# ZihanLiao/pytorch-kaldi-resnet

Measured on AMD Instinct MI355X. Metric: utterances/sec (300-frame x 80 fbank, bs256/GPU), ResNet-34 + AAM-softmax training step, higher is better.
Workload: dtype f32 (operands as 2 fp16 terms of value x 2^k, 3 cross products, f32 accumulate); 1 GPU; BASELINE configs[1]: ResNet-34 + AAM-softmax (m 0.2, s 30), 1211 speakers, 300-frame x 80 fbank, per-GPU batch 256, fwd+CE+bwd+SGD(0.9, wd 5e-4); global_batch=256, frames=300, feat_dim=80, parallelism=dp1, launch=hipGraph replay (1 graph), mfma=f16x3

## Files before the change

### include/spkhip.h

```cpp
#ifndef SPKHIP_H
#define SPKHIP_H
#include <stddef.h>
#ifdef __cplusplus
extern "C" {
#endif

int spk_version(void);
const char* spk_last_error(void);
int spk_build_flags(void);

#define SPK_IN_AFFINE_RELU 1
#define SPK_EPI_AFFINE 2
#define SPK_EPI_ADD 4
#define SPK_EPI_RELU 8
#define SPK_EPI_STATS 16
#define SPK_IN_BNBWD 64
#define SPK_EPI_BNBWD 32

#define SPK_CONV_WS 128
#define SPK_CONV_PIPE 1024

#define SPK_CONV_M16 (1 << 17)

#define SPK_WGRAD_GROUPS 2048
// ... 34 lines not shown

int spk_conv_wgrad_limits(int WN, int* max_halo_pix , int* max_tile_pix );
size_t spk_conv_wgrad_workspace(int nsplit, int ksize, int Cin, int Cout);
int spk_conv3x3_c32_stream(const float* in, const float* wpk, float* out, const float* in_scale, const float* in_shift, float* stats,
                           int B, int H, int W, int flags, const unsigned* in_amax, unsigned* out_amax, int nblocks, void* stream);
int spk_conv1x1_stream(const float* in, const float* wpk, float* out, const float* in_scale, const float* in_shift,
                       const float* epi_add, const unsigned* add_mask, const float* bn_raw, const unsigned* bn_mask,
                       const float* bn4, float* stats, long long P, int C, int flags, const unsigned* in_amax, unsigned* out_amax,
                       int nblocks, void* stream);
int spk_conv1x1_stream_rows(int nblocks, int C);
int spk_wgrad_reduce(const float* partial, float* dw, int nslab, int ksize, int Cin, int Cout, int accumulate, void* stream);
int spk_conv_wgrad(const float* x, const float* dy, float* dw, float* partial, const float* in_scale,
                   const float* in_shift, int B, int IH, int IW, int Cin, int OH, int OW, int Cout, int ksize, int stride,
                   int TH, int TW, int WN, int nsplit, int flags, int accumulate, int split , const unsigned* dy_amax , const unsigned* x_amax , void* stream);

#define SPK_PTR_ADD_MASK 1
#define SPK_PTR_BN_MASK 2
#define SPK_PTR_IN_MASK 4
#define SPK_PTR_IN_ACT 8
#define SPK_PTR_BN_ACT 16
#define SPK_PTR_SIDE_DZ 32
int spk_conv_variant_of(int MT, int NT, int split, int flags, int ptrs);
int spk_wgrad_variant_of(int ksize, int stride, int TH, int TW, int WN, int split, int flags);

int spk_stem_fwd_blocks(int B, int F, int T);
int spk_stem_conv_fwd(const float* x, const float* w, float* out, float* stats, const float* epi_scale,
                      const float* epi_shift, int B, int F, int T, int flags,
                      unsigned* amax_out , void* stream);
int spk_stem_conv_fwd_len(const float* x, const float* w, float* out, float* stats, const float* epi_scale,
                          const float* epi_shift, int B, int F, int T, int flags, unsigned* amax_out, const int* len ,
                          void* stream);
int spk_stem_wgrad_blocks(int B, int F, int T);
int spk_stem_conv_wgrad(const float* x, const float* draw, float* dw, float* partial, int B, int F, int T,
                        int accumulate, void* stream);
int spk_stem_stats(const float* x, const float* w, float* stats, int B, int F, int T, void* stream);
int spk_stem_fwd_apply(const float* x, const float* w, const float* scale, const float* shift, float* raw_out, float* act_out,
                       unsigned* mask_out, unsigned* amax_out, int B, int F, int T, void* stream);
int spk_stem_bwd_wgrad(const float* x, const float* d, const float* raw, const float* mean, const float* invstd,
                       const float* scale, const float* shift, const float* coef, float* dw, float* partial, int B, int F, int T,
                       int accumulate, void* stream);

int spk_bn_stats_blocks(long long N, int C);
int spk_bn_stats_partial(const float* x, float* partial , long long N, int C, void* stream);
size_t spk_bn_finalize_workspace(int nblk, int C);
int spk_bn_finalize(const float* partial, int nblk, int C, double count, const float* gamma, const float* beta,
                    float* running_mean, float* running_var, long long* num_batches_tracked, float* mean, float* invstd,
// ... 221 lines not shown
```

### pytorch-kaldi-resnet_amd/csrc/conv_kernel.h

```cpp
#pragma once
#include "spk_common.h"
#include <type_traits>

#ifndef STAGE_U
#define STAGE_U 4
#endif
#ifndef CONV_NT
#define CONV_NT 3
#endif
static __device__ __forceinline__ void conv_st(float* p, f32x4 v) {
    if constexpr ((CONV_NT & 1) != 0) __builtin_nontemporal_store(v, (f32x4*)p);
    else *(f32x4*)p = v;
}
template <int BIT>
static __device__ __forceinline__ f32x4 conv_ld(const float* p) {
    if constexpr ((CONV_NT & BIT) != 0) return __builtin_nontemporal_load((const f32x4*)p);
    else return *(const f32x4*)p;
}
#ifndef STAGE_U2
#define STAGE_U2 2
#endif
#ifndef STAGE_U2_C32
#define STAGE_U2_C32 4
#endif

#define SPK_SPLIT_CK 16
template <int SPLIT, int CKP = SPK_SPLIT_CK>
struct ConvCfg {
    static_assert(CKP == SPK_SPLIT_CK || (SPLIT == 3 && CKP == 32), "plane width: 16, or 32 in the f16x3 mode");
    static constexpr int NTERM = SPLIT == 3 ? 2 : 3;
    static constexpr int MAXSUM = SPLIT == 9 ? 4 : (SPLIT == 6 ? 2 : 1);
    static constexpr int CK = SPLIT ? CKP : 32;
    static constexpr int TPP = CK / 4;
    static constexpr int PPP = 256 / TPP;
    static constexpr int KG = CK / 16;
    static constexpr int LP4 = SPLIT ? (NTERM * CK * 2 + 16) / 16 : 9;
};

struct ConvArgs {
    const float* in;
    const float* wpk;
    float* out;
    const float* in_scale;
    const float* in_shift;
    const float* epi_scale;
    const float* epi_shift;
// ... 38 lines not shown
           (a.in_act ? SPK_PTR_IN_ACT : 0) | (a.bn_act ? SPK_PTR_BN_ACT : 0) | (a.side_dz ? SPK_PTR_SIDE_DZ : 0);
}

#define PIPE_D 3
#ifndef PIPE16_D
#define PIPE16_D 3
#endif
#ifndef PIPE16_D_CONV
#define PIPE16_D_CONV 3
#endif
#ifndef PIPE_VPM
#define PIPE_VPM 6
#endif
#ifdef CONV_STAMPS
#define CONV_STAMP_BLOCKS 4096
static __device__ unsigned long long g_conv_stamps[CONV_STAMP_BLOCKS][16];
#define STAMP(i) do { if (threadIdx.x == 0 && blockIdx.x < CONV_STAMP_BLOCKS) g_conv_stamps[blockIdx.x][i] = __builtin_amdgcn_s_memtime(); } while (0)
#else
#define STAMP(i) do { } while (0)
#endif
#define SPK_FL_ADDMASK (1 << 20)
#define SPK_FL_BNMASK (1 << 21)
#define SPK_FL_INMASK (1 << 22)
template <int MT, int NT, bool BNBWD, int SPLIT, bool PIPE, bool BITS = false, bool PRE = false, bool M16 = false, int FL = -1, int CKP = SPK_SPLIT_CK>
static __device__ __forceinline__ void conv_body(const ConvArgs& a) {
    using Cfg = ConvCfg<SPLIT, CKP>;
    static_assert(CKP == SPK_SPLIT_CK || (BNBWD && !PIPE), "32-channel planes: the fused BatchNorm-backward form of conv_mfma_kernel");
    constexpr int CK = Cfg::CK, TPP = Cfg::TPP, PPP = Cfg::PPP, LP4 = Cfg::LP4, NTERM = Cfg::NTERM;
    static_assert(!M16 || (PIPE && !BNBWD && SPLIT == 3), "M16: the pipelined f16x3 kernel with a plain or pair input");
    extern __shared__ __attribute__((aligned(16))) float lds[];
    const int tid = threadIdx.x, lane = tid & 63;
    const int wave = __builtin_amdgcn_readfirstlane(tid >> 6);
    const int r = lane & 31, h = lane >> 5;
    auto pix_of_row16 = [](int row) {
        const int q = (row + 12) & 15;
        return ((q & 7) << 1) | (q >> 3);
    };
    float sig = 1.f, inv_sig = 1.f, inv_wsig = 1.f;
    if constexpr (SPLIT == 3) {
        sig = a.in_amax ? spk_sigma_from_amax_bits(*a.in_amax) : a.in_sigma;
        inv_sig = 1.f / sig;
        inv_wsig = 1.f / spk_sigma_from_amax_bits(*a.w_amax);
    }
    float side_mx = 0.f;

    int bid = blockIdx.x;
    {
        const int n = a.nblocks, q = n >> 3, rr = n & 7, xcd = bid & 7, slot = bid >> 3;
        bid = (xcd < rr ? xcd * (q + 1) : rr * (q + 1) + (xcd - rr) * q) + slot;
    }
// ... 77 lines not shown
            dst[0] = t0;
            dst[CK / 4] = t1;
        }
    };
    auto store_px_q = [&](float* plane, int p, int qd, f32x4 w) {
        if constexpr (SPLIT == 0) {
            *(f32x4*)(plane + p * (LP4 * 4) + qd * 4) = w;
        } else if constexpr (SPLIT == 3) {
            uint2 t0, t1;
            split2h(w, sig, t0, t1);
            store_pair_q(plane, p, qd, t0, t1);
        } else {
            uint2 t0, t1, t2;
            split3(w, t0, t1, t2);
            uint2* dst = (uint2*)plane + p * (LP4 * 2) + qd;
            dst[0] = t0;
            dst[CK / 4] = t1;
            dst[CK / 2] = t2;
        }
    };
    auto store_pair = [&](float* plane, int p, uint2 t0, uint2 t1) { store_pair_q(plane, p, quad, t0, t1); };
    auto store_px = [&](float* plane, int p, f32x4 w) { store_px_q(plane, p, quad, w); };

    auto stage_chunk_wide = [&](int ch) {
        const int tppk = TPP * a.kc;
        const int qk = tid & (tppk - 1);
        const int pl = qk / TPP, qd = qk & (TPP - 1);
        const int prowk = tid / tppk, pppk = 256 / tppk;
        const int c = (ch * a.kc + pl) * CK + qd * 4;
        float* ldsp = lds + pl * plane_floats;
        f32x4 sc = {1.f, 1.f, 1.f, 1.f}, sh = {0.f, 0.f, 0.f, 0.f};
        if (flags & SPK_IN_AFFINE_RELU) {
            sc = *(const f32x4*)(a.in_scale + c);
            sh = *(const f32x4*)(a.in_shift + c);
        }
        constexpr int U = STAGE_U;
        for (int base = prowk; base < halo_pix; base += pppk * U) {
            f32x4 v[U];
            bool inb[U];
#pragma unroll
            for (int u = 0; u < U; ++u) {
                int p = base + pppk * u;
                p = p < halo_pix ? p : halo_pix - 1;
                const int hy = (int)__umulhi((unsigned)p, a.halo_w_magic);
                const int hx = p - hy * a.halo_w;
                const int iy = iy0 + hy, ix = ix0 + hx;
                inb[u] = iy >= 0 && iy < a.IH && ix >= 0 && ix < a.IW;
                const unsigned pi = inb[u] ? (unsigned)((iy * a.IWp + ix) * a.ips) : pi_safe_p;
                v[u] = *(const f32x4*)(img_in_p + pi * (unsigned)a.Cin + (unsigned)c);
            }
#pragma unroll
            for (int u = 0; u < U; ++u) {
                const int p = base + pppk * u;
                f32x4 w = v[u];
                if (flags & SPK_IN_AFFINE_RELU) {
                    w = w * sc + sh;
                    w[0] = fmaxf(w[0], 0.f);
                    w[1] = fmaxf(w[1], 0.f);
                    w[2] = fmaxf(w[2], 0.f);
                    w[3] = fmaxf(w[3], 0.f);
                }
                if (!inb[u]) w = (f32x4){0.f, 0.f, 0.f, 0.f};
                if constexpr (SPLIT == 3) {
                    if (flags & SPK_IN_PRESPLIT) {
                        uint2 t0, t1;
                        spk_pair_unpack(w, t0, t1);
                        if (p < halo_pix) store_pair_q(ldsp, p, qd, t0, t1);
                        continue;
                    }
                }
                if (p < halo_pix) store_px_q(ldsp, p, qd, w);
            }
        }
    };

    auto stage_chunk = [&](int ch) {
        if constexpr (!BNBWD && !PIPE) {
#ifndef CONV_NO_WIDE_STAGE
            if (a.kc > 1) {
                stage_chunk_wide(ch);
                return;
            }
#endif
        }
        for (int pl = 0; pl < a.kc; ++pl) {
            const int c = (ch * a.kc + pl) * CK + quad * 4;
            float* ldsp = lds + pl * plane_floats;
            f32x4 sc = {1.f, 1.f, 1.f, 1.f}, sh = {0.f, 0.f, 0.f, 0.f};
            if (flags & SPK_IN_AFFINE_RELU) {
                sc = *(const f32x4*)(a.in_scale + c);
                sh = *(const f32x4*)(a.in_shift + c);
            }
            if constexpr (BNBWD) {
                const f32x4 mu = *(const f32x4*)(a.in_bn4 + c), is = *(const f32x4*)(a.in_bn4 + a.Cin + c);
                const f32x4 bsc = *(const f32x4*)(a.in_bn4 + 2 * a.Cin + c), bsh = *(const f32x4*)(a.in_bn4 + 3 * a.Cin + c);
                const f32x4 k1 = *(const f32x4*)(a.in_coef + c), m1 = *(const f32x4*)(a.in_coef + a.Cin + c);
// ... 34 lines not shown
#pragma unroll
                            for (int k = 0; k < 4; ++k) dz[k] = m[k] > 0.f ? v[u][k] : 0.f;
                        }
                        f32x4 w = k1 * (dz - m1 - ((rw[u] - mu) * is) * m2);
                        if (!inb[u]) w = (f32x4){0.f, 0.f, 0.f, 0.f};
                        if (p < halo_pix) {
                            f32x4 side = w;
                            if constexpr (SPLIT == 3) {
                                uint2 t0, t1;
                                split2h(w, sig, t0, t1);
                                store_pair(ldsp, p, t0, t1);
                                if (flags & SPK_SIDE_PRESPLIT) side = spk_pair_pack(t0, t1);
                            } else
                                store_px(ldsp, p, w);
                            if (owner && core[u]) {
                                conv_st(img_draw + off[u], side);
                                if (has_side_dz) conv_st(img_dz + off[u], dz);
                                side_mx = fmaxf(side_mx, spk_finite_amax4(w));
                            }
                        }
                    }
                }
            } else {
                constexpr int U = STAGE_U;
#ifdef ABL_NO_STAGE
                for (int base = prow; base < 0; base += PPP * U) {
#else
                for (int base = prow; base < halo_pix; base += PPP * U) {
#endif
                    f32x4 v[U];
                    bool inb[U];
#pragma unroll
                    for (int u = 0; u < U; ++u) {
                        int p = base + PPP * u;
                        p = p < halo_pix ? p : halo_pix - 1;
                        const int hy = (int)__umulhi((unsigned)p, a.halo_w_magic);
                        const int hx = p - hy * a.halo_w;
                        const int iy = iy0 + hy, ix = ix0 + hx;
                        inb[u] = iy >= 0 && iy < a.IH && ix >= 0 && ix < a.IW;
                        const unsigned pi = inb[u] ? (unsigned)((iy * a.IWp + ix) * a.ips) : pi_safe_p;
                        v[u] = *(const f32x4*)(img_in_p + pi * (unsigned)a.Cin + (unsigned)c);
                    }
#pragma unroll
                    for (int u = 0; u < U; ++u) {
                        const int p = base + PPP * u;
                        f32x4 w = v[u];
                        if (flags & SPK_IN_AFFINE_RELU) {
// ... 521 lines not shown
                                                                                          acc[i][j], 0, 0, 0);
                                    else
                                        acc[i][j] = __builtin_amdgcn_mfma_f32_32x32x16_bf16(__builtin_bit_cast(bf16x8, aq[sa][i]),
                                                                                           __builtin_bit_cast(bf16x8, bc[sb][j]),
                                                                                           acc[i][j], 0, 0, 0);
                                }
                            }
                        __builtin_amdgcn_sched_barrier(0);
#pragma unroll
                        for (int s = 0; s < NTERM; ++s) {
#ifdef ABL_NO_ALOAD
                            asm volatile("" : "+v"(aq[s][i]) : "s"(o_next));
#else
                            aq[s][i] = lds4[lbase[i] + o_next + s * (CK / 8)];
#endif
                        }
                    }
                    __builtin_amdgcn_sched_barrier(0);
                };
                load_b(b0, a.tap_w[0], a.tap_g[0]);
                if (ch == 0) STAMP(0);
                __syncthreads();
                if (ch < 2) STAMP(1 + 4 * ch);
                stage_chunk(ch);
                if (ch < 2) STAMP(2 + 4 * ch);
                __syncthreads();
                if (ch < 2) STAMP(3 + 4 * ch);
                load_b(b1, a.tap_w[min(1, last)], a.tap_g[min(1, last)]);
                load_a(aq, a.tap_off[0], 0);
                int o1 = a.tap_off[min(1, last)], w2 = a.tap_w[min(2, last)], g2 = a.tap_g[min(2, last)];
                int t = 0;
                for (; t + 2 < a.ntaps; t += 3) {
                    const int i2 = min(t + 2, last), i3 = min(t + 3, last), i4 = min(t + 4, last), i5 = min(t + 5, last);
                    const int o2 = a.tap_off[i2], w3 = a.tap_w[i3], g3 = a.tap_g[i3];
                    const int o3 = a.tap_off[i3], w4 = a.tap_w[i4], g4 = a.tap_g[i4];
                    const int o4 = a.tap_off[i4], w5 = a.tap_w[i5], g5 = a.tap_g[i5];
                    step(b0, b2, o1, w2, g2);
                    step(b1, b0, o2, w3, g3);
                    step(b2, b1, o3, w4, g4);
                    o1 = o4;
                    w2 = w5;
                    g2 = g5;
                }
                if (t < a.ntaps) {
                    step(b0, b2, o1, w2, g2);
                    if (t + 1 < a.ntaps) step(b1, b0, a.tap_off[last], a.tap_w[last], a.tap_g[last]);
                }
                if (ch < 2) STAMP(4 + 4 * ch);
            }
        }
    }

// ... 233 lines not shown
    }
    if (flags & SPK_EPI_STATS) {
#pragma unroll
        for (int off = Q; off < 64; off <<= 1) {
#pragma unroll
            for (int c = 0; c < 4; ++c) {
                ssum[c] += __shfl_xor(ssum[c], off, 64);
                ssq[c] += __shfl_xor(ssq[c], off, 64);
            }
        }
        if (lane < Q) {
            float* dst = a.stats + ((size_t)(ptile * 4 + wave) * a.Cout + n0 + lane * 4) * 2;
            *(f32x4*)dst = (f32x4){ssum[0], ssq[0], ssum[1], ssq[1]};
            *(f32x4*)(dst + 4) = (f32x4){ssum[2], ssq[2], ssum[3], ssq[3]};
        }
    }
}

template <int MT, int NT, bool BNBWD, int SPLIT, int FL = -1, int CKP = SPK_SPLIT_CK>
__global__ __launch_bounds__(256) void conv_mfma_kernel(ConvArgs a) {
    conv_body<MT, NT, BNBWD, SPLIT, false, false, false, false, FL, CKP>(a);
}

template <int MT, int NT, bool BNBWD, bool BITS = false, bool PRE = false, bool M16 = false, int FL = -1>
__global__ __launch_bounds__(256, 2) void conv_pipe_kernel(ConvArgs a) {
    conv_body<MT, NT, BNBWD, 3, true, BITS, PRE, M16, FL>(a);
}
```

### pytorch-kaldi-resnet_amd/csrc/conv_mfma.hip

```cpp
#include "conv_kernel.h"

int spk_launch_conv_split(const ConvArgs& a, size_t lds_bytes, int MT, int NT, int split, int ck, hipStream_t st);
int spk_launch_conv_pipe(const ConvArgs& a, size_t lds_bytes, int MT, int NT, hipStream_t st);
int spk_launch_conv_ws(const ConvArgs& a, int MT, int NT, int WC, int split, int lp4, hipStream_t st);

template <int MT, int NT>
static int launch_conv(const ConvArgs& a, size_t lds_bytes, hipStream_t st) {
    if (a.flags & SPK_IN_BNBWD)
        hipLaunchKernelGGL((conv_mfma_kernel<MT, NT, true, 0>), dim3(a.nblocks), dim3(256), lds_bytes, st, a);
    else if (a.flags & SPK_EPI_WMASK)
        hipLaunchKernelGGL((conv_mfma_kernel<MT, NT, false, 0, SPK_EPI_WMASK>), dim3(a.nblocks), dim3(256), lds_bytes, st, a);
    else
        hipLaunchKernelGGL((conv_mfma_kernel<MT, NT, false, 0>), dim3(a.nblocks), dim3(256), lds_bytes, st, a);
    SPK_LAUNCH_CHECK("spk_conv_mfma");
    return 0;
}

static int conv_mfma_entry(const float* in, const float* wpk, float* out, const float* in_scale,
                             const float* in_shift, const float* epi_scale, const float* epi_shift,
                             const float* epi_add, const float* in_raw, const float* in_act, const float* in_bn4,
                             const float* in_coef, const unsigned* in_mask, const unsigned* bn_mask, const unsigned* add_mask, float* side_draw,
                             float* side_dz,
                             const float* bn_raw,
                             const float* bn_act, const float* bn4, float* stats, int B, int IH, int IW, int Cin, int OH,
                             int OW, int OHf, int OWf, int Cout, int IS, int OS, int ooy, int oox, int ntaps,
                             const int* tap_dy, const int* tap_dx, const int* tap_w, int TH, int TW, int MT,
                             int NT, int kc, int ips, int flags, int split, const unsigned* in_amax, unsigned* out_amax,
                             unsigned* side_amax, const int* wlen, void* stream) {
    SPK_REQUIRE(in && wpk && out, "spk_conv_mfma: null pointer");
    SPK_REQUIRE(!(flags & SPK_EPI_WMASK) || wlen, "spk_conv_mfma: SPK_EPI_WMASK needs wlen (spk_conv_mfma_len)");
    SPK_REQUIRE(!wlen || (flags & SPK_EPI_WMASK), "spk_conv_mfma_len: wlen given without SPK_EPI_WMASK");
    SPK_REQUIRE(!(flags & SPK_EPI_WMASK) || !(flags & (SPK_IN_BNBWD | SPK_EPI_BNBWD | SPK_IN_PRESPLIT | SPK_SIDE_PRESPLIT | SPK_CONV_WS)),
                "spk_conv_mfma_len: SPK_EPI_WMASK is implemented for the forward forms only (no IN_BNBWD, EPI_BNBWD, IN_PRESPLIT, "
                "SIDE_PRESPLIT or CONV_WS)");
    SPK_REQUIRE(B > 0 && IH > 0 && IW > 0 && OH > 0 && OW > 0, "spk_conv_mfma: empty tensor");
    SPK_REQUIRE(Cin % 32 == 0 && Cin > 0, "spk_conv_mfma: Cin=%d must be a multiple of 32", Cin);
    const int ws_wc = (flags & SPK_CONV_WS) ? 1 << ((flags >> 8) & 3) : 1;
    SPK_REQUIRE(ws_wc <= 4, "spk_conv_mfma: bad wave layout");
    SPK_REQUIRE(NT >= 1 && Cout % (32 * NT * ws_wc) == 0, "spk_conv_mfma: Cout=%d not a multiple of 32*NT*WC (NT=%d, WC=%d)", Cout, NT, ws_wc);
    SPK_REQUIRE(ntaps >= 1 && ntaps <= 9, "spk_conv_mfma: ntaps=%d out of range", ntaps);
    SPK_REQUIRE(split == 0 || split == 3 || split == 6 || split == 9,
                "spk_conv_mfma: split=%d (0 = fp32 operands, 6 / 9 = bf16 cross terms, 3 = fp16 two-term operands)", split);
    const bool ck32 = (flags & SPK_CONV_CK32) != 0;
    SPK_REQUIRE(!ck32 || (split == 3 && Cin == 32 && (flags & SPK_IN_BNBWD) && kc == 1 && !(flags & (SPK_CONV_WS | SPK_CONV_PIPE))),
                "spk_conv_mfma: CONV_CK32 (32-channel planes) exists for the fused BatchNorm-backward form of conv_mfma_kernel at Cin = 32 in the "
                "f16x3 mode");
    flags &= ~SPK_CONV_CK32;
    const int ck = split ? (ck32 ? 32 : SPK_SPLIT_CK) : 32;
    const int nterm = split == 3 ? 2 : 3;
    const int lp4 = split ? (nterm * ck * 2 + 16) / 16 : 9;
    const int kgrp = split ? ck / 16 : 1;
    SPK_REQUIRE(kc >= 1 && ntaps * kc * kgrp <= (ck32 ? 18 : 9) && Cin % (ck * kc) == 0, "spk_conv_mfma: kc=%d incompatible with ntaps=%d, Cin=%d", kc, ntaps, Cin);
    SPK_REQUIRE(TH >= 1 && TW >= 1 && TH * TW <= 128 * MT / ws_wc, "spk_conv_mfma: tile %dx%d exceeds %d pixels (MT=%d)", TH, TW, 128 * MT / ws_wc, MT);
    SPK_REQUIRE(IS >= 1 && OS >= 1 && ooy >= 0 && oox >= 0, "spk_conv_mfma: bad strides/offsets");
    SPK_REQUIRE((OH - 1) * OS + ooy < OHf && (OW - 1) * OS + oox < OWf, "spk_conv_mfma: logical grid exceeds the output tensor");
    SPK_REQUIRE((long long)B * OHf * OWf * Cout < 2147483647LL && (long long)B * IH * IW * Cin < 2147483647LL * 4,
                "spk_conv_mfma: tensor too large for 32-bit element offsets");
    SPK_REQUIRE((long long)IH * IW * Cin < 2147483647LL, "spk_conv_mfma: one image exceeds 32-bit element offsets");
    SPK_REQUIRE(!(flags & SPK_IN_AFFINE_RELU) || (in_scale && in_shift), "spk_conv_mfma: IN_AFFINE_RELU needs scale/shift");
    SPK_REQUIRE(!(flags & SPK_EPI_AFFINE) || (epi_scale && epi_shift), "spk_conv_mfma: EPI_AFFINE needs scale/shift");
    SPK_REQUIRE(!(flags & SPK_EPI_ADD) || epi_add, "spk_conv_mfma: EPI_ADD needs epi_add");
    SPK_REQUIRE(!(flags & SPK_EPI_STATS) || stats, "spk_conv_mfma: EPI_STATS needs a stats buffer");
    SPK_REQUIRE(!(flags & SPK_IN_BNBWD) || (in_raw && in_bn4 && in_coef && side_draw && !(flags & SPK_IN_AFFINE_RELU)),
                "spk_conv_mfma: IN_BNBWD needs in_raw, in_bn4, in_coef and side_draw (and excludes IN_AFFINE_RELU)");
    SPK_REQUIRE(!(flags & SPK_IN_BNBWD) || (IS == 1 && OS == 1 && ips == 1 && OH == IH && OW == IW && OHf == IH && OWf == IW),
                "spk_conv_mfma: IN_BNBWD is defined for stride-1 data gradients (input and output grids coincide)");
    SPK_REQUIRE(!(flags & SPK_EPI_BNBWD) || ((flags & SPK_EPI_STATS) && bn_raw && bn4),
                "spk_conv_mfma: EPI_BNBWD needs EPI_STATS, bn_raw and bn4");
    SPK_REQUIRE(split != 3 || in_amax, "spk_conv_mfma: the f16x3 operand mode needs in_amax (slot with the float bits of the staged tensor's absmax or of an upper bound)");
    SPK_REQUIRE(!(flags & SPK_IN_PRESPLIT) || (split == 3 && !(flags & (SPK_IN_AFFINE_RELU | SPK_IN_BNBWD | SPK_CONV_WS))),
// ... 73 lines not shown
            const long long off = (long long)a.tap_w[t] * (Cin >> 4) * nterm * (Cout >> 5) * 256;
            SPK_REQUIRE(off < 2147483647LL, "spk_conv_mfma: packed weight offset overflows");
            a.tap_boff[t] = (int)off;
        }
        return spk_launch_conv_ws(a, MT, NT, ws_wc, split, lp4, st);
#endif
    }
    if (flags & SPK_CONV_PIPE) {
        SPK_REQUIRE(split == 3 && kc == 1 && ntaps == 9, "spk_conv_mfma: the pipelined kernel needs f16x3 operands, 9 taps and kc = 1");
        SPK_REQUIRE(!(flags & SPK_IN_BNBWD) || !in_act || in_mask,
                    "spk_conv_mfma: the pipelined kernel takes the ReLU mask of a fused BatchNorm backward as sign bits or recomputes it");
        SPK_REQUIRE(a.halo_h * a.halo_w <= 9 * 64, "spk_conv_mfma: the pipelined kernel stages at most 576 halo pixels (%d x %d)", a.halo_h, a.halo_w);
        size_t lds2 = (2 * (size_t)a.halo_h * a.halo_w + 1) * lp4 * 16;
        if (lds2 < red_bytes) lds2 = red_bytes;
        SPK_REQUIRE(lds2 <= 160 * 1024, "spk_conv_mfma: two halo tiles %dx%d need %zu B of LDS", a.halo_h, a.halo_w, lds2);
        if (flags & SPK_CONV_M16) {
            SPK_REQUIRE(!(flags & SPK_IN_BNBWD), "spk_conv_mfma: CONV_M16 excludes the fused BatchNorm backward");
            SPK_REQUIRE(a.halo_h * a.halo_w <= 8 * 64, "spk_conv_mfma: CONV_M16 stages at most 512 halo pixels (%d x %d)", a.halo_h, a.halo_w);
            SPK_REQUIRE((Cin / SPK_SPLIT_CK) % 2 == 0, "spk_conv_mfma: CONV_M16 walks the 16-channel planes in pairs");
        }
        a.flags = flags & ~SPK_CONV_PIPE;
        return spk_launch_conv_pipe(a, lds2, MT, NT, st);
    }
    if (split) return spk_launch_conv_split(a, lds_bytes, MT, NT, split, ck, st);
#define CASE(M, N) if (MT == M && NT == N) return launch_conv<M, N>(a, lds_bytes, st)
    CASE(1, 1); CASE(2, 1); CASE(3, 1); CASE(4, 1);
    CASE(1, 2); CASE(2, 2); CASE(3, 2); CASE(4, 2);
    CASE(1, 4); CASE(2, 4);
#undef CASE
    spk_set_error("spk_conv_mfma: unsupported tile config MT=%d NT=%d", MT, NT);
    return -1;
}

extern "C" int spk_conv_variant_of(int MT, int NT, int split, int flags, int ptrs) {
    if (flags & SPK_CONV_WS) return -1;
    const int ck = (flags & SPK_CONV_CK32) ? 32 : SPK_SPLIT_CK;
    flags &= ~SPK_CONV_CK32;
    if (flags & SPK_CONV_PIPE) return split == 3 ? spk_pipe_variant_of(MT, NT, flags & ~SPK_CONV_PIPE, ptrs) : -1;
    return split ? spk_split_variant_of(MT, NT, split, ck, flags, ptrs) : -1;
}

extern "C" int spk_conv_mfma(const float* in, const float* wpk, float* out, const float* in_scale,
                             const float* in_shift, const float* epi_scale, const float* epi_shift,
                             const float* epi_add, const float* in_raw, const float* in_act, const float* in_bn4,
                             const float* in_coef, const unsigned* in_mask, const unsigned* bn_mask, const unsigned* add_mask, float* side_draw,
                             float* side_dz, const float* bn_raw, const float* bn_act, const float* bn4, float* stats, int B, int IH,
                             int IW, int Cin, int OH, int OW, int OHf, int OWf, int Cout, int IS, int OS, int ooy, int oox, int ntaps,
                             const int* tap_dy, const int* tap_dx, const int* tap_w, int TH, int TW, int MT,
                             int NT, int kc, int ips, int flags, int split, const unsigned* in_amax, unsigned* out_amax,
                             unsigned* side_amax, void* stream) {
    return conv_mfma_entry(in, wpk, out, in_scale, in_shift, epi_scale, epi_shift, epi_add, in_raw, in_act, in_bn4, in_coef, in_mask,
                           bn_mask, add_mask, side_draw, side_dz, bn_raw, bn_act, bn4, stats, B, IH, IW, Cin, OH, OW, OHf, OWf, Cout, IS,
                           OS, ooy, oox, ntaps, tap_dy, tap_dx, tap_w, TH, TW, MT, NT, kc, ips, flags, split, in_amax, out_amax,
                           side_amax, nullptr, stream);
}

extern "C" int spk_conv_mfma_len(const float* in, const float* wpk, float* out, const float* in_scale,
                                 const float* in_shift, const float* epi_scale, const float* epi_shift,
                                 const float* epi_add, const float* in_raw, const float* in_act, const float* in_bn4,
                                 const float* in_coef, const unsigned* in_mask, const unsigned* bn_mask, const unsigned* add_mask,
                                 float* side_draw, float* side_dz, const float* bn_raw, const float* bn_act, const float* bn4,
                                 float* stats, int B, int IH, int IW, int Cin, int OH, int OW, int OHf, int OWf, int Cout, int IS,
// ... 10 lines not shown
```

### pytorch-kaldi-resnet_amd/csrc/conv_split.hip

```cpp
#include "conv_kernel.h"

constexpr int FLV_BNBWD2 = SPK_IN_BNBWD | SPK_SIDE_PRESPLIT | SPK_EPI_STATS | SPK_EPI_BNBWD | SPK_FL_INMASK;
constexpr int FLV_BNBWD1 = SPK_IN_BNBWD | SPK_SIDE_PRESPLIT | SPK_EPI_ADD | SPK_EPI_STATS | SPK_EPI_BNBWD | SPK_FL_ADDMASK | SPK_FL_BNMASK;
constexpr int FLV_FWD_AFF = SPK_IN_AFFINE_RELU | SPK_EPI_STATS;
constexpr int FLV_FWD = SPK_EPI_STATS;
constexpr int FLV_DGRAD_PAIR = SPK_IN_PRESPLIT;
constexpr int FLV_DGRAD_ADD = SPK_EPI_ADD;

static constexpr bool split_has_fl(int MT, int NT, int ck, int fl) {
    const bool t21 = MT == 2 && NT == 1, t12 = MT == 1 && NT == 2, t22 = MT == 2 && NT == 2, t32 = MT == 3 && NT == 2;
    if (ck == 32) return (t21 || (MT == 1 && NT == 1)) && (fl == FLV_BNBWD1 || fl == FLV_BNBWD2);
    switch (fl) {
        case FLV_BNBWD1: case FLV_BNBWD2: return t21;
        case FLV_FWD_AFF: return t21 || t12 || t22;
        case FLV_FWD: return t21 || t12 || t22 || t32 || (MT == 1 && NT == 4);
        case FLV_DGRAD_PAIR: case FLV_DGRAD_ADD: return t21 || t22 || t32;
    }
    return false;
}

int spk_split_variant_of(int MT, int NT, int split, int ck, int flags, int ptrs) {
#ifdef SPK_NO_FL_VARIANTS
    return -1;
#else
    if (!spk_fl_variants_enabled() || split != 3 || (flags & SPK_EPI_WMASK)) return -1;
    int fl = flags;
    if (flags & SPK_IN_BNBWD) {
        if (ptrs & (SPK_PTR_IN_ACT | SPK_PTR_BN_ACT | SPK_PTR_SIDE_DZ)) return -1;
        fl |= ((ptrs & SPK_PTR_ADD_MASK) ? SPK_FL_ADDMASK : 0) | ((ptrs & SPK_PTR_BN_MASK) ? SPK_FL_BNMASK : 0) |
              ((ptrs & SPK_PTR_IN_MASK) ? SPK_FL_INMASK : 0);
    } else if (ptrs & (SPK_PTR_ADD_MASK | SPK_PTR_BN_MASK | SPK_PTR_BN_ACT)) {
        return -1;
    }
    return split_has_fl(MT, NT, ck, fl) ? fl : -1;
#endif
}

#define FL_CASE(V, CK)                                                                                                                \
    case V:                                                                                                                           \
        if constexpr (split_has_fl(MT, NT, CK, V)) {                                                                                  \
            hipLaunchKernelGGL((conv_mfma_kernel<MT, NT, ((V) & SPK_IN_BNBWD) != 0, 3, V, CK>), dim3(a.nblocks), dim3(256), lds_bytes, st, a); \
            return true;                                                                                                              \
        }                                                                                                                             \
        break;

template <int MT, int NT>
static bool launch_fl_ck32(int fl, const ConvArgs& a, size_t lds_bytes, hipStream_t st) {
#ifndef SPK_NO_FL_VARIANTS
    switch (fl) {
        FL_CASE(FLV_BNBWD2, 32)
        FL_CASE(FLV_BNBWD1, 32)
    }
#endif
    return false;
}

template <int MT, int NT>
static int launch_split_ck32(const ConvArgs& a, size_t lds_bytes, hipStream_t st) {
    const int fl = spk_split_variant_of(MT, NT, 3, 32, a.flags, conv_ptr_pattern(a));
    if (fl < 0)
        hipLaunchKernelGGL((conv_mfma_kernel<MT, NT, true, 3, -1, 32>), dim3(a.nblocks), dim3(256), lds_bytes, st, a);
// ... 20 lines not shown
    return false;
}
#undef FL_CASE

template <int MT, int NT, int SPLIT>
static int launch_split(const ConvArgs& a, size_t lds_bytes, hipStream_t st) {
    const int fl = spk_split_variant_of(MT, NT, SPLIT, SPK_SPLIT_CK, a.flags, conv_ptr_pattern(a));
    if (fl >= 0) {
        if (!launch_fl<MT, NT>(fl, a, lds_bytes, st)) {
            spk_set_error("spk_conv_mfma: no instance of flag variant 0x%x for MT=%d NT=%d", fl, MT, NT);
            return -1;
        }
    } else if (a.flags & SPK_IN_BNBWD) {
        hipLaunchKernelGGL((conv_mfma_kernel<MT, NT, true, SPLIT>), dim3(a.nblocks), dim3(256), lds_bytes, st, a);
    } else if (a.flags & SPK_EPI_WMASK) {
        hipLaunchKernelGGL((conv_mfma_kernel<MT, NT, false, SPLIT, SPK_EPI_WMASK>), dim3(a.nblocks), dim3(256), lds_bytes, st, a);
    } else {
        hipLaunchKernelGGL((conv_mfma_kernel<MT, NT, false, SPLIT>), dim3(a.nblocks), dim3(256), lds_bytes, st, a);
    }
    SPK_LAUNCH_CHECK("spk_conv_mfma(split)");
    return 0;
}

int spk_launch_conv_split(const ConvArgs& a, size_t lds_bytes, int MT, int NT, int split, int ck, hipStream_t st) {
    if (ck == 32) {
        if (MT == 2 && NT == 1) return launch_split_ck32<2, 1>(a, lds_bytes, st);
        if (MT == 1 && NT == 1) return launch_split_ck32<1, 1>(a, lds_bytes, st);
        spk_set_error("spk_conv_mfma: 32-channel planes are instantiated for MT=2 / MT=1 with NT=1, not MT=%d NT=%d", MT, NT);
        return -1;
    }
#define CASE(M, N)                                                      \
    if (MT == M && NT == N) {                                           \
        if (split == 3) return launch_split<M, N, 3>(a, lds_bytes, st); \
        if (split == 6) return launch_split<M, N, 6>(a, lds_bytes, st); \
        return launch_split<M, N, 9>(a, lds_bytes, st);                 \
    }
    CASE(1, 1) CASE(2, 1) CASE(3, 1) CASE(4, 1) CASE(1, 2) CASE(2, 2) CASE(3, 2) CASE(1, 4)
#undef CASE
    spk_set_error("spk_conv_mfma: unsupported split tile config MT=%d NT=%d", MT, NT);
    return -1;
}

#ifdef CONV_STAMPS
extern "C" int spk_debug_stamps(unsigned long long* out, int nblocks) {
    if (nblocks < 0) {
        void* p = nullptr;
        if (hipGetSymbolAddress(&p, HIP_SYMBOL(g_conv_stamps)) != hipSuccess) return -1;
// ... 7 lines not shown
```

### pytorch-kaldi-resnet_amd/csrc/spk_common.h

```cpp
#pragma once
#include <hip/hip_runtime.h>
#include <stdint.h>

typedef float f32x4 __attribute__((ext_vector_type(4)));
typedef float f32x16 __attribute__((ext_vector_type(16)));

void spk_set_error(const char* fmt, ...);
#define SPK_REQUIRE(cond, ...)                 \
    do {                                       \
        if (!(cond)) {                         \
            spk_set_error(__VA_ARGS__);        \
            return -1;                         \
        }                                      \
    } while (0)
#define SPK_LAUNCH_CHECK(name)                                                          \
    do {                                                                                \
        hipError_t e__ = hipGetLastError();                                             \
        if (e__ != hipSuccess) {                                                        \
            spk_set_error("%s: launch failed: %s", name, hipGetErrorString(e__));       \
            return (int)e__;                                                            \
        }                                                                               \
    } while (0)

enum {
// ... 11 lines not shown
    SPK_SIDE_PRESPLIT = 1 << 15,
    SPK_DY_PRESPLIT = 1 << 16,
    SPK_CONV_M16 = 1 << 17,
    SPK_WGRAD_NOSHIFT = 1 << 18,
    SPK_WGRAD_M16 = 1 << 19,
    SPK_CONV_CK32 = 1 << 23,
    SPK_EPI_WMASK = 1 << 24
};

static inline int spk_ceil_div(int a, int b) { return (a + b - 1) / b; }

int spk_diar_check(const char* who, const long long* rec_off, int R, long long Ntot, long long* tab);

enum {
    SPK_PTR_ADD_MASK = 1,
    SPK_PTR_BN_MASK = 2,
    SPK_PTR_IN_MASK = 4,
    SPK_PTR_IN_ACT = 8,
    SPK_PTR_BN_ACT = 16,
    SPK_PTR_SIDE_DZ = 32
};
bool spk_fl_variants_enabled();
int spk_split_variant_of(int MT, int NT, int split, int ck, int flags, int ptrs);
int spk_pipe_variant_of(int MT, int NT, int flags, int ptrs);
int spk_wgrad_split_variant_of(int ksize, int WN, int split, int flags, int halo_pix);

typedef __bf16 bf16x8 __attribute__((ext_vector_type(8)));
#ifdef __HIPCC__
static __device__ __forceinline__ unsigned pack_bf16x2(float lo, float hi, float& rlo, float& rhi) {
    const __bf16 a = (__bf16)lo, b = (__bf16)hi;
    rlo = lo - (float)a;
    rhi = hi - (float)b;
    return (unsigned)__builtin_bit_cast(unsigned short, a) | ((unsigned)__builtin_bit_cast(unsigned short, b) << 16);
}
static __device__ __forceinline__ void split3(f32x4 w, uint2& t0, uint2& t1, uint2& t2) {
    float r0, r1, r2, r3, q0, q1, q2, q3;
    t0.x = pack_bf16x2(w[0], w[1], r0, r1);
    t0.y = pack_bf16x2(w[2], w[3], r2, r3);
    t1.x = pack_bf16x2(r0, r1, q0, q1);
    t1.y = pack_bf16x2(r2, r3, q2, q3);
    t2.x = pack_bf16x2(q0, q1, r0, r1);
    t2.y = pack_bf16x2(q2, q3, r2, r3);
}
typedef _Float16 f16x8 __attribute__((ext_vector_type(8)));
#define SPK_F16_ACT_SIGMA 64.0f
typedef _Float16 f16x4 __attribute__((ext_vector_type(4)));
// ... 53 lines not shown
```

### pytorch-kaldi-resnet_amd/hip.py

```python
import ctypes
import os

import torch

_HERE = os.path.dirname(os.path.abspath(__file__))
LIB_PATH = os.environ.get("SPK_LIB", os.path.join(_HERE, "libspkhip.so"))

IN_AFFINE_RELU, EPI_AFFINE, EPI_ADD, EPI_RELU, EPI_STATS, EPI_BNBWD, IN_BNBWD, CONV_WS = 1, 2, 4, 8, 16, 32, 64, 128
CONV_PIPE = 1024
WGRAD_GROUPS = 2048
IN_PRESPLIT, SIDE_PRESPLIT, DY_PRESPLIT = 1 << 14, 1 << 15, 1 << 16
CONV_M16 = 1 << 17
CONV_CK32 = 1 << 23
WGRAD_NOSHIFT = 1 << 18
WGRAD_M16 = 1 << 19
EPI_WMASK = 1 << 24
PTR_ADD_MASK, PTR_BN_MASK, PTR_IN_MASK, PTR_IN_ACT, PTR_BN_ACT, PTR_SIDE_DZ = 1, 2, 4, 8, 16, 32
MASK_NONE, MASK_ACT, MASK_RAW, MASK_BITS = 0, 1, 2, 3

_P = ctypes.c_void_p
_I = ctypes.c_int
_L = ctypes.c_longlong
_F = ctypes.c_float
_D = ctypes.c_double
_IP = ctypes.POINTER(ctypes.c_int)

_SIGS = {
    "spk_pack_conv_weight": [_P, _P, _I, _I, _I, _I, _I, _P],
    "spk_pack_conv_weight_split": [_P, _P, _I, _I, _I, _I, _I, _I, _P],
    "spk_pack_job_bytes": [],
    "spk_build_flags": [],
    "spk_pack_conv_weights_batched": [_P, _I, _I, _I, _P],
    "spk_conv_mfma": [_P] * 21 + [_I] * 14 + [_IP, _IP, _IP] + [_I] * 8 + [_P, _P, _P, _P],
    "spk_conv_mfma_len": [_P] * 21 + [_I] * 14 + [_IP, _IP, _IP] + [_I] * 8 + [_P, _P, _P, _P, _P],
    "spk_conv3x3_c32_stream": [_P] * 6 + [_I] * 4 + [_P, _P, _I, _P],
    "spk_conv1x1_stream": [_P] * 11 + [_L, _I, _I, _P, _P, _I, _P],
    "spk_conv1x1_stream_rows": [_I, _I],
    "spk_conv_wgrad": [_P] * 6 + [_I] * 16 + [_P, _P, _P],
    "spk_conv_wgrad_limits": [_I, _IP, _IP],
    "spk_wgrad_reduce": [_P, _P, _I, _I, _I, _I, _I, _P],
    "spk_conv_variant_of": [_I, _I, _I, _I, _I],
    "spk_wgrad_variant_of": [_I, _I, _I, _I, _I, _I, _I],
    "spk_stem_fwd_blocks": [_I, _I, _I],
    "spk_stem_conv_fwd": [_P] * 6 + [_I] * 4 + [_P, _P],
    "spk_stem_conv_fwd_len": [_P] * 6 + [_I] * 4 + [_P, _P, _P],
    "spk_stem_wgrad_blocks": [_I, _I, _I],
    "spk_stem_conv_wgrad": [_P] * 4 + [_I] * 4 + [_P],
    "spk_stem_stats": [_P] * 3 + [_I] * 3 + [_P],
    "spk_stem_fwd_apply": [_P] * 8 + [_I] * 3 + [_P],
    "spk_stem_bwd_wgrad": [_P] * 10 + [_I] * 4 + [_P],
    "spk_bn_stats_blocks": [_L, _I],
    "spk_bn_stats_partial": [_P, _P, _L, _I, _P],
    "spk_bn_finalize": [_P, _I, _I, _D] + [_P] * 9 + [_F, _F, _P, _P, _P, _P],
    "spk_bn_eval_coeffs": [_P] * 6 + [_I, _F, _P],
    "spk_bn_apply": [_P] * 8 + [_L, _I, _I, _P, _P],
    "spk_bn_bwd_reduce": [_P] * 8 + [_L, _I, _I, _P, _P],
    "spk_bn_bwd_finalize": [_P, _I, _I, _D] + [_P] * 5 + [_I, _P, _P, _P, _P, _P, _P, _P],
    "spk_bn_bwd_apply": [_P] * 10 + [_L, _I, _I, _P, _P, _P],
    "spk_absmax": [_P, _P, _L, _P],
    "spk_bnbwd_estimate": [_P, _P, _P, _I, _P, _P, _P, _P],
    "spk_f16_window_count": [_P, _P, _P, _L, _I, _P, _I, _P, _P],
    "spk_affine_estimate": [_P, _P, _I, _P, _P, _P],
    "spk_se_chunks": [_L],
    "spk_se_squeeze": [_P, _P, _P, _I, _I, _I, _I, _P, _P],
    "spk_se_excite": [_P] * 8 + [_I] * 5 + [_P, _P],
# ... 163 lines not shown
```

Before: 5661 utt/s.

## Add register-prefetch staging and 32-channel plane forward for strided f16x3 convs

Adds a stage selector for non-pipelined f16x3 forward convolutions with statistics on stride-2 inputs. For MT=1 NT=4 it picks a prefetching kernel that issues the next chunk's global loads into registers before the MFMA loop and writes them to LDS after the barrier, so load latency overlaps compute. For Cin=32 1x1 MT=1 NT=2 it switches to a 32-channel-plane kernel with kc=1. Both raise register pressure and add more kernel instances to compile.

```diff
diff --git a/include/spkhip.h b/include/spkhip.h
--- a/include/spkhip.h
+++ b/include/spkhip.h
@@ -80,6 +80,7 @@
 #define SPK_PTR_SIDE_DZ 32
 int spk_conv_variant_of(int MT, int NT, int split, int flags, int ptrs);
 int spk_wgrad_variant_of(int ksize, int stride, int TH, int TW, int WN, int split, int flags);
+int spk_conv_stage_of(int MT, int NT, int split, int Cin, int IS, int ips, int ntaps, int kc, int flags, int ptrs);
 
 int spk_stem_fwd_blocks(int B, int F, int T);
 int spk_stem_conv_fwd(const float* x, const float* w, float* out, float* stats, const float* epi_scale,
diff --git a/pytorch-kaldi-resnet_amd/csrc/conv_kernel.h b/pytorch-kaldi-resnet_amd/csrc/conv_kernel.h
--- a/pytorch-kaldi-resnet_amd/csrc/conv_kernel.h
+++ b/pytorch-kaldi-resnet_amd/csrc/conv_kernel.h
@@ -22,6 +22,9 @@
 #endif
 #ifndef STAGE_U2_C32
 #define STAGE_U2_C32 4
+#endif
+#ifndef STAGE_U_C32F
+#define STAGE_U_C32F 4
 #endif
 
 #define SPK_SPLIT_CK 16
@@ -106,10 +109,14 @@
 #define SPK_FL_ADDMASK (1 << 20)
 #define SPK_FL_BNMASK (1 << 21)
 #define SPK_FL_INMASK (1 << 22)
-template <int MT, int NT, bool BNBWD, int SPLIT, bool PIPE, bool BITS = false, bool PRE = false, bool M16 = false, int FL = -1, int CKP = SPK_SPLIT_CK>
+template <int MT, int NT, bool BNBWD, int SPLIT, bool PIPE, bool BITS = false, bool PRE = false, bool M16 = false, int FL = -1, int CKP = SPK_SPLIT_CK,
+          int PF = 0>
 static __device__ __forceinline__ void conv_body(const ConvArgs& a) {
     using Cfg = ConvCfg<SPLIT, CKP>;
-    static_assert(CKP == SPK_SPLIT_CK || (BNBWD && !PIPE), "32-channel planes: the fused BatchNorm-backward form of conv_mfma_kernel");
+    static_assert(CKP == SPK_SPLIT_CK || (!PIPE && (BNBWD || FL == SPK_EPI_STATS)),
+                  "32-channel planes: the fused BatchNorm-backward form of conv_mfma_kernel, and its plain forward with statistics");
+    static_assert(PF == 0 || (!PIPE && !BNBWD && SPLIT == 3 && FL == SPK_EPI_STATS && CKP == SPK_SPLIT_CK),
+                  "PF: the non-pipelined f16x3 forward with statistics on 16-channel planes");
     constexpr int CK = Cfg::CK, TPP = Cfg::TPP, PPP = Cfg::PPP, LP4 = Cfg::LP4, NTERM = Cfg::NTERM;
     static_assert(!M16 || (PIPE && !BNBWD && SPLIT == 3), "M16: the pipelined f16x3 kernel with a plain or pair input");
     extern __shared__ __attribute__((aligned(16))) float lds[];
@@ -233,7 +240,7 @@
     auto store_pair = [&](float* plane, int p, uint2 t0, uint2 t1) { store_pair_q(plane, p, quad, t0, t1); };
     auto store_px = [&](float* plane, int p, f32x4 w) { store_px_q(plane, p, quad, w); };
 
-    auto stage_chunk_wide = [&](int ch) {
+    auto stage_chunk_wide = [&](int ch, int first = 0) {
         const int tppk = TPP * a.kc;
         const int qk = tid & (tppk - 1);
         const int pl = qk / TPP, qd = qk & (TPP - 1);
@@ -246,7 +253,7 @@
             sh = *(const f32x4*)(a.in_shift + c);
         }
         constexpr int U = STAGE_U;
-        for (int base = prowk; base < halo_pix; base += pppk * U) {
+        for (int base = prowk + first; base < halo_pix; base += pppk * U) {
             f32x4 v[U];
             bool inb[U];
 #pragma unroll
@@ -283,6 +290,44 @@
                 if (p < halo_pix) store_px_q(ldsp, p, qd, w);
             }
         }
+    };
+
+    f32x4 pf[PF > 0 ? PF : 1];
+    unsigned pf_inb = 0;
+    auto pf_issue = [&](int ch) {
+        const int tppk = TPP * a.kc, qk = tid & (tppk - 1);
+        const int pl = qk / TPP, qd = qk & (TPP - 1), pppk = 256 / tppk;
+        int prowk = tid / tppk;
+        asm volatile("" : "+v"(prowk));
+        const int c = (ch * a.kc + pl) * CK + qd * 4;
+        pf_inb = 0;
+#pragma unroll
+        for (int u = 0; u < PF; ++u) {
+            int p = prowk + pppk * u;
+            p = p < halo_pix ? p : halo_pix - 1;
+            const int hy = (int)__umulhi((unsigned)p, a.halo_w_magic);
+            const int hx = p - hy * a.halo_w;
+            const int iy = iy0 + hy, ix = ix0 + hx;
+            const bool ok = iy >= 0 && iy < a.IH && ix >= 0 && ix < a.IW;
+            pf_inb |= (unsigned)ok << u;
+            const unsigned pi = ok ? (unsigned)((iy * a.IWp + ix) * a.ips) : pi_safe_p;
+            pf[u] = *(const f32x4*)(img_in_p + pi * (unsigned)a.Cin + (unsigned)c);
+        }
+    };
+    auto pf_finish = [&](int ch) {
+        const int tppk = TPP * a.kc, qk = tid & (tppk - 1);
+        const int pl = qk / TPP, qd = qk & (TPP - 1), pppk = 256 / tppk;
+        int prowk = tid / tppk;
+        asm volatile("" : "+v"(prowk));
+        float* ldsp = lds + pl * plane_floats;
+#pragma unroll
+        for (int u = 0; u < PF; ++u) {
+            const int p = prowk + pppk * u;
+            f32x4 w = pf[u];
+            if (!((pf_inb >> u) & 1u)) w = (f32x4){0.f, 0.f, 0.f, 0.f};
+            if (p < halo_pix) store_px_q(ldsp, p, qd, w);
+        }
+        stage_chunk_wide(ch, pppk * PF);
     };
 
     auto stage_chunk = [&](int ch) {
@@ -363,7 +408,7 @@
                     }
                 }
             } else {
-                constexpr int U = STAGE_U;
+                constexpr int U = (SPLIT == 3 && CKP == 32) ? STAGE_U_C32F : STAGE_U;
 #ifdef ABL_NO_STAGE
                 for (int base = prow; base < 0; base += PPP * U) {
 #else
@@ -931,12 +976,19 @@
                 if (ch == 0) STAMP(0);
                 __syncthreads();
                 if (ch < 2) STAMP(1 + 4 * ch);
-                stage_chunk(ch);
+                if constexpr (PF > 0) {
+                    if (ch == 0) pf_issue(0);
+                    pf_finish(ch);
+                } else
+                    stage_chunk(ch);
                 if (ch < 2) STAMP(2 + 4 * ch);
                 __syncthreads();
                 if (ch < 2) STAMP(3 + 4 * ch);
                 load_b(b1, a.tap_w[min(1, last)], a.tap_g[min(1, last)]);
                 load_a(aq, a.tap_off[0], 0);
+                if constexpr (PF > 0) {
+                    if (ch + 1 < nchunks) pf_issue(ch + 1);
+                }
                 int o1 = a.tap_off[min(1, last)], w2 = a.tap_w[min(2, last)], g2 = a.tap_g[min(2, last)];
                 int t = 0;
                 for (; t + 2 < a.ntaps; t += 3) {
@@ -1216,6 +1268,11 @@
     conv_body<MT, NT, BNBWD, SPLIT, false, false, false, false, FL, CKP>(a);
 }
 
+template <int MT, int NT, int PF>
+__global__ __launch_bounds__(256) void conv_mfma_pf_kernel(ConvArgs a) {
+    conv_body<MT, NT, false, 3, false, false, false, false, SPK_EPI_STATS, SPK_SPLIT_CK, PF>(a);
+}
+
 template <int MT, int NT, bool BNBWD, bool BITS = false, bool PRE = false, bool M16 = false, int FL = -1>
 __global__ __launch_bounds__(256, 2) void conv_pipe_kernel(ConvArgs a) {
     conv_body<MT, NT, BNBWD, 3, true, BITS, PRE, M16, FL>(a);
diff --git a/pytorch-kaldi-resnet_amd/csrc/conv_mfma.hip b/pytorch-kaldi-resnet_amd/csrc/conv_mfma.hip
--- a/pytorch-kaldi-resnet_amd/csrc/conv_mfma.hip
+++ b/pytorch-kaldi-resnet_amd/csrc/conv_mfma.hip
@@ -1,6 +1,6 @@
 #include "conv_kernel.h"
 
-int spk_launch_conv_split(const ConvArgs& a, size_t lds_bytes, int MT, int NT, int split, int ck, hipStream_t st);
+int spk_launch_conv_split(const ConvArgs& a, size_t lds_bytes, int MT, int NT, int split, int ck, int stage, hipStream_t st);
 int spk_launch_conv_pipe(const ConvArgs& a, size_t lds_bytes, int MT, int NT, hipStream_t st);
 int spk_launch_conv_ws(const ConvArgs& a, int MT, int NT, int WC, int split, int lp4, hipStream_t st);
 
@@ -41,11 +41,21 @@
     SPK_REQUIRE(ntaps >= 1 && ntaps <= 9, "spk_conv_mfma: ntaps=%d out of range", ntaps);
     SPK_REQUIRE(split == 0 || split == 3 || split == 6 || split == 9,
                 "spk_conv_mfma: split=%d (0 = fp32 operands, 6 / 9 = bf16 cross terms, 3 = fp16 two-term operands)", split);
-    const bool ck32 = (flags & SPK_CONV_CK32) != 0;
+    bool ck32 = (flags & SPK_CONV_CK32) != 0;
     SPK_REQUIRE(!ck32 || (split == 3 && Cin == 32 && (flags & SPK_IN_BNBWD) && kc == 1 && !(flags & (SPK_CONV_WS | SPK_CONV_PIPE))),
                 "spk_conv_mfma: CONV_CK32 (32-channel planes) exists for the fused BatchNorm-backward form of conv_mfma_kernel at Cin = 32 in the "
                 "f16x3 mode");
     flags &= ~SPK_CONV_CK32;
+    int stage = SPK_STAGE_PLAIN;
+    if (split == 3 && !ck32 && !(flags & (SPK_CONV_WS | SPK_CONV_PIPE))) {
+        const int ptrs = (add_mask ? SPK_PTR_ADD_MASK : 0) | (bn_mask ? SPK_PTR_BN_MASK : 0) | (in_mask ? SPK_PTR_IN_MASK : 0) |
+                         (in_act ? SPK_PTR_IN_ACT : 0) | (bn_act ? SPK_PTR_BN_ACT : 0) | (side_dz ? SPK_PTR_SIDE_DZ : 0);
+        stage = spk_split_stage_of(MT, NT, split, Cin, IS, ips, ntaps, kc, flags, ptrs);
+    }
+    if (stage == SPK_STAGE_CK32) {
+        ck32 = true;
+        kc = 1;
+    }
     const int ck = split ? (ck32 ? 32 : SPK_SPLIT_CK) : 32;
     const int nterm = split == 3 ? 2 : 3;
     const int lp4 = split ? (nterm * ck * 2 + 16) / 16 : 9;
@@ -165,7 +175,7 @@
         a.flags = flags & ~SPK_CONV_PIPE;
         return spk_launch_conv_pipe(a, lds2, MT, NT, st);
     }
-    if (split) return spk_launch_conv_split(a, lds_bytes, MT, NT, split, ck, st);
+    if (split) return spk_launch_conv_split(a, lds_bytes, MT, NT, split, ck, stage, st);
 #define CASE(M, N) if (MT == M && NT == N) return launch_conv<M, N>(a, lds_bytes, st)
     CASE(1, 1); CASE(2, 1); CASE(3, 1); CASE(4, 1);
     CASE(1, 2); CASE(2, 2); CASE(3, 2); CASE(4, 2);
@@ -181,6 +191,11 @@
     flags &= ~SPK_CONV_CK32;
     if (flags & SPK_CONV_PIPE) return split == 3 ? spk_pipe_variant_of(MT, NT, flags & ~SPK_CONV_PIPE, ptrs) : -1;
     return split ? spk_split_variant_of(MT, NT, split, ck, flags, ptrs) : -1;
+}
+
+extern "C" int spk_conv_stage_of(int MT, int NT, int split, int Cin, int IS, int ips, int ntaps, int kc, int flags, int ptrs) {
+    if (split != 3 || (flags & (SPK_CONV_WS | SPK_CONV_PIPE | SPK_CONV_CK32))) return SPK_STAGE_PLAIN;
+    return spk_split_stage_of(MT, NT, split, Cin, IS, ips, ntaps, kc, flags, ptrs);
 }
 
 extern "C" int spk_conv_mfma(const float* in, const float* wpk, float* out, const float* in_scale,
diff --git a/pytorch-kaldi-resnet_amd/csrc/conv_split.hip b/pytorch-kaldi-resnet_amd/csrc/conv_split.hip
--- a/pytorch-kaldi-resnet_amd/csrc/conv_split.hip
+++ b/pytorch-kaldi-resnet_amd/csrc/conv_split.hip
@@ -36,7 +36,16 @@
 #endif
 }
 
-#define FL_CASE(V, CK)                                                                                                                \
+static constexpr int split_pf_depth(int MT, int NT) { return (MT == 1 && NT == 4) ? 9 : 0; }
+
+int spk_split_stage_of(int MT, int NT, int split, int Cin, int IS, int ips, int ntaps, int kc, int flags, int ptrs) {
+    if (spk_split_variant_of(MT, NT, split, SPK_SPLIT_CK, flags, ptrs) != FLV_FWD || (IS != 2 && ips != 2)) return SPK_STAGE_PLAIN;
+    if (Cin == 32 && MT == 1 && NT == 2 && ntaps == 1 && (kc == 1 || kc == 2)) return SPK_STAGE_CK32;
+    if (split_pf_depth(MT, NT) > 0 && (kc == 1 || kc == 2 || kc == 4) && Cin / (SPK_SPLIT_CK * kc) >= 2) return SPK_STAGE_PREFETCH;
+    return SPK_STAGE_PLAIN;
+}
+
+#define FL_CASE(V, CK)                                                                                                               \
     case V:                                                                                                                           \
         if constexpr (split_has_fl(MT, NT, CK, V)) {                                                                                  \
             hipLaunchKernelGGL((conv_mfma_kernel<MT, NT, ((V) & SPK_IN_BNBWD) != 0, 3, V, CK>), dim3(a.nblocks), dim3(256), lds_bytes, st, a); \
@@ -103,7 +112,26 @@
     return 0;
 }
 
-int spk_launch_conv_split(const ConvArgs& a, size_t lds_bytes, int MT, int NT, int split, int ck, hipStream_t st) {
+int spk_launch_conv_split(const ConvArgs& a, size_t lds_bytes, int MT, int NT, int split, int ck, int stage, hipStream_t st) {
+    if (stage == SPK_STAGE_CK32) {
+        if (MT != 1 || NT != 2 || ck != 32 || a.flags != FLV_FWD) {
+            spk_set_error("spk_conv_mfma: the whole-pixel forward is instantiated for MT=1 NT=2 with statistics, not MT=%d NT=%d flags 0x%x", MT, NT, a.flags);
+            return -1;
+        }
+        hipLaunchKernelGGL((conv_mfma_kernel<1, 2, false, 3, FLV_FWD, 32>), dim3(a.nblocks), dim3(256), lds_bytes, st, a);
+        SPK_LAUNCH_CHECK("spk_conv_mfma(split, whole-pixel forward)");
+        return 0;
+    }
+    if (stage == SPK_STAGE_PREFETCH) {
+        if (MT == 1 && NT == 4 && a.flags == FLV_FWD)
+            hipLaunchKernelGGL((conv_mfma_pf_kernel<1, 4, split_pf_depth(1, 4)>), dim3(a.nblocks), dim3(256), lds_bytes, st, a);
+        else {
+            spk_set_error("spk_conv_mfma: no prefetching instance for MT=%d NT=%d flags 0x%x", MT, NT, a.flags);
+            return -1;
+        }
+        SPK_LAUNCH_CHECK("spk_conv_mfma(split, prefetching forward)");
+        return 0;
+    }
     if (ck == 32) {
         if (MT == 2 && NT == 1) return launch_split_ck32<2, 1>(a, lds_bytes, st);
         if (MT == 1 && NT == 1) return launch_split_ck32<1, 1>(a, lds_bytes, st);
diff --git a/pytorch-kaldi-resnet_amd/csrc/spk_common.h b/pytorch-kaldi-resnet_amd/csrc/spk_common.h
--- a/pytorch-kaldi-resnet_amd/csrc/spk_common.h
+++ b/pytorch-kaldi-resnet_amd/csrc/spk_common.h
@@ -57,6 +57,12 @@
 };
 bool spk_fl_variants_enabled();
 int spk_split_variant_of(int MT, int NT, int split, int ck, int flags, int ptrs);
+enum {
+    SPK_STAGE_PLAIN = 0,
+    SPK_STAGE_PREFETCH = 1,
+    SPK_STAGE_CK32 = 32
+};
+int spk_split_stage_of(int MT, int NT, int split, int Cin, int IS, int ips, int ntaps, int kc, int flags, int ptrs);
 int spk_pipe_variant_of(int MT, int NT, int flags, int ptrs);
 int spk_wgrad_split_variant_of(int ksize, int WN, int split, int flags, int halo_pix);
 
diff --git a/pytorch-kaldi-resnet_amd/hip.py b/pytorch-kaldi-resnet_amd/hip.py
--- a/pytorch-kaldi-resnet_amd/hip.py
+++ b/pytorch-kaldi-resnet_amd/hip.py
@@ -41,6 +41,7 @@
     "spk_wgrad_reduce": [_P, _P, _I, _I, _I, _I, _I, _P],
     "spk_conv_variant_of": [_I, _I, _I, _I, _I],
     "spk_wgrad_variant_of": [_I, _I, _I, _I, _I, _I, _I],
+    "spk_conv_stage_of": [_I] * 10,
     "spk_stem_fwd_blocks": [_I, _I, _I],
     "spk_stem_conv_fwd": [_P] * 6 + [_I] * 4 + [_P, _P],
     "spk_stem_conv_fwd_len": [_P] * 6 + [_I] * 4 + [_P, _P, _P],
```

Result: no change. 5668 utt/s (median of 4 runs) (+0.1%).
